# gau-nernst/pytorch-models

Measured on NVIDIA B200. Metric: ViT-B/16 img/s bf16, higher is better.
Workload: dtype bf16

## Files before the change

pytorch_models_b200/csrc/api_linear.cu:

```cuda
#include "../../include/b200enc.h"
#include "gemm.cuh"
#include "host_util.h"

using namespace b200;

namespace {

template <int kCtas, bool kFold, int kAct, bool kRes, bool kStats, bool kF8 = false, bool kPatch = false>
int launch_gemm(const CUtensorMap& ta, const CUtensorMap& tb, const CUtensorMap& tc, const GemmParams& p, int grid,
                cudaStream_t stream) {
  auto kern = gemm_bf16_kernel<kCtas, kFold, kAct, kRes, kStats, kF8, kPatch>;
  constexpr int kSmem = GemmSmem<kCtas, kRes>::kBytes;
  if (int rc = ensure_dynamic_smem(reinterpret_cast<const void*>(kern), kSmem)) return rc;
  cudaLaunchConfig_t cfg = {};
  cfg.gridDim = dim3(grid);
  cfg.blockDim = dim3(GEMM_THREADS);
  cfg.dynamicSmemBytes = kSmem;
  cfg.stream = stream;
  cudaLaunchAttribute attr[2];
  attr[0].id = cudaLaunchAttributeClusterDimension;
  attr[0].val.clusterDim.x = kCtas;
  attr[0].val.clusterDim.y = 1;
  attr[0].val.clusterDim.z = 1;
  attr[1].id = cudaLaunchAttributeProgrammaticStreamSerialization;
  attr[1].val.programmaticStreamSerializationAllowed = 1;
  cfg.attrs = attr;
  cfg.numAttrs = pdl_enabled() ? 2 : 1;
  B200_CUDA(cudaLaunchKernelEx(&cfg, kern, ta, tb, tc, p));
  return 0;
}

template <int kCtas, bool kFold, int kAct, bool kRes>
int dispatch_store(bool stats, const CUtensorMap& ta, const CUtensorMap& tb, const CUtensorMap& tc, const GemmParams& p,
                   int grid, cudaStream_t s) {
  if constexpr (kRes && !kFold) {
    if (stats) return launch_gemm<kCtas, kFold, kAct, kRes, true>(ta, tb, tc, p, grid, s);
  }
  if (stats) return set_error(-1, "b200enc_linear: stats_out needs a residual, non-folded epilogue");
  return launch_gemm<kCtas, kFold, kAct, kRes, false>(ta, tb, tc, p, grid, s);
}

template <int kCtas>
int dispatch_fp8(bool gelu, bool res, const CUtensorMap& ta, const CUtensorMap& tb, const CUtensorMap& tc, const GemmParams& p,
                 int grid, cudaStream_t s) {
  if (gelu && res) return set_error(-1, "b200enc_linear: FP8 variant: GELU and residual cannot be combined");
  if (gelu) return launch_gemm<kCtas, false, 1, false, false, true>(ta, tb, tc, p, grid, s);
  if (res) return launch_gemm<kCtas, false, 0, true, false, true>(ta, tb, tc, p, grid, s);
  return launch_gemm<kCtas, false, 0, false, false, true>(ta, tb, tc, p, grid, s);
}

template <int kCtas>
int dispatch_epilogue(int sel, bool stats, const CUtensorMap& ta, const CUtensorMap& tb,
                      const CUtensorMap& tc, const GemmParams& p, int grid, cudaStream_t s) {
  switch (sel) {
    case 0: return dispatch_store<kCtas, false, 0, false>(stats, ta, tb, tc, p, grid, s);
    case 1: return dispatch_store<kCtas, false, 0, true>(stats, ta, tb, tc, p, grid, s);
    case 2: return dispatch_store<kCtas, false, 1, false>(stats, ta, tb, tc, p, grid, s);
    case 3: return dispatch_store<kCtas, false, 1, true>(stats, ta, tb, tc, p, grid, s);
    case 4: return dispatch_store<kCtas, true, 0, false>(stats, ta, tb, tc, p, grid, s);
    case 5: return dispatch_store<kCtas, true, 0, true>(stats, ta, tb, tc, p, grid, s);
// ... 83 lines not shown
  B200_CHECK_ARG(a->ldx >= 8 && a->ldw >= K && a->ldo >= N,
                 "b200enc_linear: leading dimension smaller than the row length");
  B200_CHECK_ARG((a->colsum == nullptr) == (a->rowstats == nullptr),
                 "b200enc_linear: colsum and rowstats must be given together (LayerNorm fold)");
  if (a->colsum) {
    const int want = (K + GEMM_STAT_SLICE - 1) / GEMM_STAT_SLICE;
    B200_CHECK_ARG(a->rowstats_parts == 0 || (a->rowstats_parts == want && want <= 12),
                   "b200enc_linear: rowstats_parts=%d must be 0 or ceil(K/128)=%d (<= 12)", a->rowstats_parts, want);
  }
  B200_CHECK_ARG((reinterpret_cast<uintptr_t>(a->bias) & 15u) == 0 && (reinterpret_cast<uintptr_t>(a->colsum) & 15u) == 0,
                 "b200enc_linear: bias / colsum must be 16-byte aligned");
  if (a->residual) {
    B200_CHECK_ARG(a->ldr >= N && a->ldr % 8 == 0 && a->res_batch_stride % 8 == 0 &&
                       (reinterpret_cast<uintptr_t>(a->residual) & 15u) == 0,
                   "b200enc_linear: residual must be 16-byte aligned with strides that are multiples of 8");
  }
  const bool fold = a->colsum != nullptr;
  const bool gelu = (a->flags & B200ENC_LINEAR_GELU) != 0;
  const bool gelu_tanh = (a->flags & B200ENC_LINEAR_GELU_TANH) != 0;
  const bool relu = (a->flags & B200ENC_LINEAR_RELU) != 0;
  const bool silu = (a->flags & B200ENC_LINEAR_SILU) != 0;
  B200_CHECK_ARG(int(gelu) + int(gelu_tanh) + int(relu) + int(silu) <= 1,
                 "b200enc_linear: at most one activation flag may be set");
  constexpr int kLinearFlags =
      B200ENC_LINEAR_GELU | B200ENC_LINEAR_GELU_TANH | B200ENC_LINEAR_RELU | B200ENC_LINEAR_SILU | B200ENC_LINEAR_FP8;
  B200_CHECK_ARG((a->flags & ~kLinearFlags) == 0, "b200enc_linear: flags=%d has bits outside the documented set (0x%x)",
                 a->flags, kLinearFlags);
  const bool res = a->residual != nullptr;
  const bool stats = a->stats_out != nullptr;

  int ctas = M > GEMM_BM ? 2 : 1;
  if (ctas == 2 && K <= 1024) {
    const long long tn = (N + GEMM_BN - 1) / GEMM_BN;
    const long long t2 = (long long)((M + 2 * GEMM_BM - 1) / (2 * GEMM_BM)) * tn * batches;
    const long long t1 = (long long)((M + GEMM_BM - 1) / GEMM_BM) * tn * batches;
    const long long s2 = sm_count() / 2, s1 = sm_count();
    const double cost2 = double((t2 + s2 - 1) / s2);
    const double cost1 = double((t1 + s1 - 1) / s1) * 1.15;
    if (cost1 < cost2 * 0.97) ctas = 1;
  }
  CUtensorMap ta, tb, tc;
  int rc;
  if (fp8) {
    if ((rc = make_tmap_u8(&ta, a->x, K, M, batches, a->ldx, batches > 1 ? a->x_batch_stride : (long long)M * a->ldx,
                           2 * GEMM_BK, GEMM_BM, 128)))
      return rc;
    if ((rc = make_tmap_u8(&tb, a->w, K, N, 0, a->ldw, 0, 2 * GEMM_BK, GEMM_BN / ctas, 128))) return rc;
  } else {
    if ((rc = make_tmap_bf16(&ta, a->x, K, M, batches, a->ldx, batches > 1 ? a->x_batch_stride : (long long)M * a->ldx,
                             GEMM_BK, GEMM_BM, 128)))
      return rc;
    if ((rc = make_tmap_bf16(&tb, a->w, K, N, 0, a->ldw, 0, GEMM_BK, GEMM_BN / ctas, 128))) return rc;
  }
  if ((rc = make_tmap_bf16(&tc, a->out, N, M, batches, a->ldo,
                           batches > 1 ? a->out_batch_stride : (long long)M * a->ldo, 64, 32, 128)))
    return rc;

  GemmParams p = {};
  p.M = M;
  p.N = N;
  p.K = K;
  p.batches = batches;
  p.tiles_m = (M + GEMM_BM * ctas - 1) / (GEMM_BM * ctas);
  p.tiles_n = (N + GEMM_BN - 1) / GEMM_BN;
  p.bias = a->bias;
  p.colsum = a->colsum;
  p.rowstats = reinterpret_cast<const float2*>(a->rowstats);
  p.stat_parts = a->rowstats_parts;
  p.ln_eps = a->ln_eps;
  p.stats_out = reinterpret_cast<float2*>(a->stats_out);
  p.stats_rows = a->stats_rows_per_batch > 0 ? a->stats_rows_per_batch : M;
  p.stats_off = a->stats_row_offset;
  B200_CHECK_ARG(a->stats_row_offset >= 0 && p.stats_rows >= M + a->stats_row_offset,
                 "b200enc_linear: stats_rows_per_batch=%d cannot hold M=%d rows at offset %d", p.stats_rows, M,
                 a->stats_row_offset);
  p.res = reinterpret_cast<const __nv_bfloat16*>(a->residual);
  p.res_batch_stride = a->res_batch_stride;
  p.ldr = a->ldr;
  p.acc_scale = a->acc_scale;
  p.abort_word = abort_word();

  const long long total = (long long)p.tiles_m * p.tiles_n * batches;
  const int slots = sm_count() / ctas;
  const int grid = int(total < slots ? total : slots) * ctas;
  cudaStream_t s = reinterpret_cast<cudaStream_t>(stream);
  if (fp8) {
    if (ctas == 2) return dispatch_fp8<2>(gelu, res, ta, tb, tc, p, grid, s);
    return dispatch_fp8<1>(gelu, res, ta, tb, tc, p, grid, s);
  }
  const int sel = (silu ? 32 : 0) | (relu ? 16 : 0) | (gelu_tanh ? 8 : 0) | (fold ? 4 : 0) | (gelu ? 2 : 0) | (res ? 1 : 0);
  if (ctas == 2) return dispatch_epilogue<2>(sel, stats, ta, tb, tc, p, grid, s);
  return dispatch_epilogue<1>(sel, stats, ta, tb, tc, p, grid, s);
}
```

pytorch_models_b200/csrc/gemm.cuh:

```cuda
#pragma once
#include "ptx.cuh"

namespace b200 {

constexpr int GEMM_BM = 128;
constexpr int GEMM_BN = 256;
constexpr int GEMM_BK = 64;
constexpr int GEMM_THREADS = 320;
constexpr int GEMM_EPI_WARPS = 8;
#ifndef GEMM_STAGES_2CTA
#define GEMM_STAGES_2CTA 5
#endif
constexpr int GEMM_STAT_SLICE = 128;
constexpr int GEMM_A_BYTES = GEMM_BM * GEMM_BK * 2;
constexpr int GEMM_B_BYTES = GEMM_BN * GEMM_BK * 2;
constexpr int GEMM_STAGE_BYTES = GEMM_A_BYTES + GEMM_B_BYTES;
constexpr int GEMM_STG_BYTES = 32 * 128;
constexpr int GEMM_SMEM_COLVEC = GEMM_EPI_WARPS * 2 * 128 * 4;
template <int kCtas, bool kRes = false>
struct GemmSmem {
  static constexpr int kStages = kCtas == 2 ? (kRes ? 4 : GEMM_STAGES_2CTA) : 3;
  static constexpr int kBRows = GEMM_BN / kCtas;
  static constexpr int kStageBytes = GEMM_A_BYTES + kBRows * GEMM_BK * 2;
  static constexpr int kRing = kStages * kStageBytes;
// ... 50 lines not shown
}

__device__ __forceinline__ float2 silu_fast2(float2 x) {
  const float2 w = __fmul2_rn(x, make_float2(-1.4426950408889634f, -1.4426950408889634f));
  const float2 den = __fadd2_rn(make_float2(fast_exp2(w.x), fast_exp2(w.y)), make_float2(1.0f, 1.0f));
  return make_float2(x.x * __frcp_rn(den.x), x.y * __frcp_rn(den.y));
}

template <int kCtas, bool kFold, int kAct, bool kRes, bool kStats, bool kF8 = false, bool kPatch = false>
__global__ void __launch_bounds__(GEMM_THREADS, 1)
gemm_bf16_kernel(const __grid_constant__ CUtensorMap tmA, const __grid_constant__ CUtensorMap tmB,
                 const __grid_constant__ CUtensorMap tmC, const GemmParams p) {
  extern __shared__ __align__(1024) uint8_t smem[];
  const uint32_t smem_base = smem_u32(smem);
  using SM = GemmSmem<kCtas, kRes>;
  const uint32_t ring = smem_base;
  float* colvec = reinterpret_cast<float*>(smem + SM::kRing + SM::kStg);
  const uint32_t bars = smem_base + SM::kRing + SM::kStg + GEMM_SMEM_COLVEC;
  constexpr int kStages = SM::kStages;
  constexpr int kBRows = SM::kBRows;
  constexpr int kStageBytes = SM::kStageBytes;
  constexpr int kTileM = GEMM_BM * kCtas;
  constexpr bool kTmaOut = !kPatch;
  auto full_bar = [&](int s) { return bars + 8u * s; };
  auto empty_bar = [&](int s) { return bars + 8u * (kStages + s); };
  auto tfull_bar = [&](int a) { return bars + 8u * (2 * kStages + a); };
  auto tempty_bar = [&](int a) { return bars + 8u * (2 * kStages + 2 + a); };
  volatile uint32_t* tmem_slot = reinterpret_cast<volatile uint32_t*>(
      smem + SM::kRing + SM::kStg + GEMM_SMEM_COLVEC + 8 * (2 * kStages + 4));

  const int hw_warp = threadIdx.x >> 5;
  const int warp = (hw_warp + 2) % (GEMM_THREADS / 32);
  const int lane = threadIdx.x & 31;
  const uint32_t cta_rank = kCtas == 2 ? cluster_ctarank() : 0u;

  if (smem_base & 1023u) {
    if (threadIdx.x == 0 && p.abort_word != nullptr) *reinterpret_cast<volatile unsigned int*>(p.abort_word) = 0xB200A116u;
    return;
  }
  WaitCtx wctx = make_wait_ctx(p.abort_word);
  if (threadIdx.x == 0) {
    for (int s = 0; s < kStages; ++s) {
      mbar_init(full_bar(s), 1);
      mbar_init(empty_bar(s), 1);
    }
    for (int a = 0; a < 2; ++a) {
      mbar_init(tfull_bar(a), 1);
      mbar_init(tempty_bar(a), GEMM_EPI_WARPS * kCtas);
    }
    fence_mbar_init();
    tma_prefetch_desc(&tmA);
    tma_prefetch_desc(&tmB);
    if (kTmaOut) tma_prefetch_desc(&tmC);
  }
  if (warp == 1) {
    if (kCtas == 2) {
      tmem_alloc_2cta<512>(smem_u32(const_cast<uint32_t*>(tmem_slot)));
      tmem_relinquish_2cta();
    } else {
      tmem_alloc<512>(smem_u32(const_cast<uint32_t*>(tmem_slot)));
      tmem_relinquish();
    }
  }
  tc_fence_before();
  if (kCtas == 2) cluster_sync_all(); else __syncthreads();
  tc_fence_after();
  const uint32_t tmem_base = *tmem_slot;
  griddep_launch_dependents();
  griddep_wait();

  constexpr int kBKe = kF8 ? 2 * GEMM_BK : GEMM_BK;
  const int num_kb = (p.K + kBKe - 1) / kBKe;
  const int tiles_per_batch = p.tiles_m * p.tiles_n;
  const int total_tiles = tiles_per_batch * p.batches;
  const int first_tile = blockIdx.x / kCtas;
  const int tile_step = gridDim.x / kCtas;

  if (warp == 0) {
    uint32_t stage = 0, phase = 0;
    for (int tile = first_tile; tile < total_tiles; tile += tile_step) {
      const int b = tile / tiles_per_batch;
      const int r = tile - b * tiles_per_batch;
      const int m0 = (r / p.tiles_n) * kTileM + int(cta_rank) * GEMM_BM;
      const int n0 = (r % p.tiles_n) * GEMM_BN + int(cta_rank) * kBRows;
      for (int kb = 0; kb < num_kb; ++kb) {
        mbar_wait(empty_bar(stage), phase ^ 1u, wctx);
        const uint32_t sa = ring + stage * kStageBytes;
        if (elect_one()) {
          if (kCtas == 2) {
            const uint32_t leader_full = map_to_cta(full_bar(stage), 0);
            if (cta_rank == 0) mbar_expect_tx(full_bar(stage), 2 * kStageBytes);
            tma_load_3d_2cta(&tmA, leader_full, sa, kb * kBKe, m0, b);
            tma_load_2d_2cta(&tmB, leader_full, sa + GEMM_A_BYTES, kb * kBKe, n0);
          } else if (kPatch) {
            const int tm = r / p.tiles_n;
            mbar_expect_tx(full_bar(stage), kStageBytes);
            tma_load_4d(&tmA, full_bar(stage), sa, 0, (b * 3 + (kb >> 2)) * p.pt_hp + 8 * (tm / p.pt_nw16), (kb & 3) * 4,
                        16 * (tm % p.pt_nw16));
            tma_load_2d(&tmB, full_bar(stage), sa + GEMM_A_BYTES, kb * kBKe, n0);
          } else {
            mbar_expect_tx(full_bar(stage), kStageBytes);
            tma_load_3d(&tmA, full_bar(stage), sa, kb * kBKe, m0, b);
            tma_load_2d(&tmB, full_bar(stage), sa + GEMM_A_BYTES, kb * kBKe, n0);
          }
        }
        __syncwarp();
        if (++stage == kStages) {
          stage = 0;
          phase ^= 1u;
        }
      }
    }
  } else if (warp == 1) {
    if (cta_rank == 0) {
      constexpr uint32_t idesc = kF8 ? make_idesc_e4m3(kTileM, GEMM_BN) : make_idesc_bf16(kTileM, GEMM_BN, 0, 0);
      uint32_t stage = 0, phase = 0, acc = 0, acc_phase = 0;
      for (int tile = first_tile; tile < total_tiles; tile += tile_step) {
        mbar_wait(tempty_bar(acc), acc_phase ^ 1u, wctx);
        tc_fence_after();
        const uint32_t d_tmem = tmem_base + acc * GEMM_BN;
        for (int kb = 0; kb < num_kb; ++kb) {
          mbar_wait(full_bar(stage), phase, wctx);
          tc_fence_after();
          const uint32_t sa = ring + stage * kStageBytes;
          const uint64_t da = kPatch ? make_smem_desc_sw32(sa, 256, 1024) : make_smem_desc_sw128(sa, 16, 1024);
          constexpr uint32_t kAStep = kPatch ? 16u : 2u;
          const uint64_t db = make_smem_desc_sw128(sa + GEMM_A_BYTES, 16, 1024);
          if (elect_one()) {
#pragma unroll
            for (int k = 0; k < GEMM_BK / 16; ++k) {
              if (kF8) {
                if (kCtas == 2)
                  umma_ss_f8_2cta(d_tmem, da + kAStep * k, db + 2u * k, idesc, (kb | k) != 0 ? 1u : 0u);
                else
                  umma_ss_f8(d_tmem, da + kAStep * k, db + 2u * k, idesc, (kb | k) != 0 ? 1u : 0u);
              } else if (kCtas == 2)
                umma_ss_2cta(d_tmem, da + kAStep * k, db + 2u * k, idesc, (kb | k) != 0 ? 1u : 0u);
              else
                umma_ss(d_tmem, da + kAStep * k, db + 2u * k, idesc, (kb | k) != 0 ? 1u : 0u);
            }
            if (kCtas == 2) umma_commit_2cta(empty_bar(stage), 3); else umma_commit(empty_bar(stage));
            if (kb == num_kb - 1) {
              if (kCtas == 2) umma_commit_2cta(tfull_bar(acc), 3); else umma_commit(tfull_bar(acc));
            }
          }
          __syncwarp();
          if (++stage == kStages) {
            stage = 0;
            phase ^= 1u;
          }
        }
        acc ^= 1u;
        if (acc == 0) acc_phase ^= 1u;
      }
    }
  } else {
    const int q = hw_warp & 3;
    const int hf = (warp - 2) >> 2;
    const uint32_t stg = smem_base + SM::kRing + (warp - 2) * (SM::kStgBufs * GEMM_STG_BYTES);
    uint8_t* stg_ptr = smem + SM::kRing + (warp - 2) * (SM::kStgBufs * GEMM_STG_BYTES);
    float* cv_b = colvec + (warp - 2) * 256;
    float* cv_s = cv_b + 128;
    const int n_slices = (p.N + GEMM_STAT_SLICE - 1) / GEMM_STAT_SLICE;
    uint32_t acc = 0, acc_phase = 0;
    const uint32_t tempty_leader0 = kCtas == 2 ? map_to_cta(tempty_bar(0), 0) : tempty_bar(0);
    for (int tile = first_tile; tile < total_tiles; tile += tile_step) {
      const int b = tile / tiles_per_batch;
      const int r = tile - b * tiles_per_batch;
      const int m0 = (r / p.tiles_n) * kTileM + int(cta_rank) * GEMM_BM;
      const int n0 = (r % p.tiles_n) * GEMM_BN;
      const int pt_ph0 = kPatch ? 8 * ((r / p.tiles_n) / p.pt_nw16) : 0;
      const int pt_pw0 = kPatch ? 16 * ((r / p.tiles_n) % p.pt_nw16) : 0;
      auto tile_row = [&](int rt, bool& ok) {
        if (kPatch) {
          const int ph = pt_ph0 + (rt & 7), pw = pt_pw0 + (rt >> 3);
          ok = ph < p.pt_hp && pw < p.pt_wp;
          return ph * p.pt_wp + pw;
        }
        ok = m0 + rt < p.M;
        return m0 + rt;
      };
      bool row_ok;
      const int row = tile_row(q * 32 + lane, row_ok);
      const int nh = n0 + hf * 128;

      float4 my_b = make_float4(0.f, 0.f, 0.f, 0.f), my_s = make_float4(0.f, 0.f, 0.f, 0.f);
      if (nh + 4 * lane < p.N) {
        if (p.bias != nullptr) my_b = __ldg(reinterpret_cast<const float4*>(p.bias + nh) + lane);
        if (kFold) my_s = __ldg(reinterpret_cast<const float4*>(p.colsum + nh) + lane);
      }
      float2 st_full = make_float2(0.0f, 1.0f);
      constexpr int kMaxParts = 12;
      float2 st_part[kMaxParts];
      if (kFold && row_ok) {
        const long long grow = (long long)b * p.M + row;
        if (p.stat_parts == 0) {
          st_full = __ldg(p.rowstats + grow);
        } else {
#pragma unroll
          for (int t = 0; t < kMaxParts; ++t)
            if (t < p.stat_parts) st_part[t] = __ldg(p.rowstats + grow * p.stat_parts + t);
        }
      }
      uint4 rres[2][8];
      if (kRes) {
// ... 191 lines not shown
```

pytorch_models_b200/csrc/host_util.cu:

```cuda
#include <cstdlib>
#include "host_util.h"

#include <string.h>

#include <mutex>
#include <unordered_map>

namespace b200 {

static thread_local char g_err[512] = "";

char* last_error_buf() { return g_err; }

int set_error(int code, const char* fmt, ...) {
  va_list ap;
  va_start(ap, fmt);
  vsnprintf(g_err, sizeof(g_err), fmt, ap);
  va_end(ap);
  return code;
}

typedef CUresult (*EncodeTiledFn)(CUtensorMap*, CUtensorMapDataType, cuuint32_t, void*, const cuuint64_t*,
                                  const cuuint64_t*, const cuuint32_t*, const cuuint32_t*, CUtensorMapInterleave,
                                  CUtensorMapSwizzle, CUtensorMapL2promotion, CUtensorMapFloatOOBfill);
// ... 115 lines not shown
  if (row_stride % 16 != 0) return set_error(-1, "row stride %llu bytes is not a multiple of 16", (unsigned long long)row_stride);
  const int rank = batches == 0 ? 2 : 3;
  if (rank == 3 && batch_stride % 16 != 0)
    return set_error(-1, "batch stride %llu bytes is not a multiple of 16", (unsigned long long)batch_stride);
  const uint64_t dims[3] = {inner, rows, batches == 0 ? 1 : batches};
  const uint64_t strides[2] = {row_stride, batch_stride};
  const uint32_t box[3] = {box_inner, box_rows, 1};
  return make_tmap_bf16_nd(out, base, rank, dims, strides, box, swizzle_bytes, 1);
}

namespace {
constexpr int kMaxDevices = 64;
}

int sm_count() {
  static int counts[kMaxDevices] = {0};
  int dev = 0;
  if (cudaGetDevice(&dev) != cudaSuccess || dev < 0 || dev >= kMaxDevices) return 148;
  int n = counts[dev];
  if (n) return n;
  if (cudaDeviceGetAttribute(&n, cudaDevAttrMultiProcessorCount, dev) != cudaSuccess || n <= 0) n = 148;
  counts[dev] = n;
  return n;
}

bool pdl_enabled() {
  static const bool on = [] {
    const char* e = getenv("B200ENC_PDL");
    return !(e != nullptr && e[0] == '0');
  }();
  return on;
}

int ensure_dynamic_smem(const void* kernel, int bytes) {
  struct Key {
    const void* k;
    int dev;
    bool operator==(const Key& o) const { return k == o.k && dev == o.dev; }
  };
  struct KeyHash {
    size_t operator()(const Key& x) const { return std::hash<const void*>()(x.k) ^ (size_t(x.dev) * 0x9E3779B1u); }
  };
  static std::mutex mu;
  static std::unordered_map<Key, int, KeyHash> done;
  int dev = 0;
  B200_CUDA(cudaGetDevice(&dev));
  {
    std::lock_guard<std::mutex> lk(mu);
    auto it = done.find(Key{kernel, dev});
    if (it != done.end() && it->second >= bytes) return 0;
  }
  B200_CUDA(cudaFuncSetAttribute(kernel, cudaFuncAttributeMaxDynamicSharedMemorySize, bytes));
  std::lock_guard<std::mutex> lk(mu);
  done[Key{kernel, dev}] = bytes;
  return 0;
}

static unsigned int* g_abort_host = nullptr;

unsigned int* abort_word() {
  static std::once_flag once;
  std::call_once(once, [] {
    void* p = nullptr;
    if (cudaHostAlloc(&p, 64, cudaHostAllocMapped | cudaHostAllocPortable) == cudaSuccess && p != nullptr) {
      memset(p, 0, 64);
      g_abort_host = static_cast<unsigned int*>(p);
// ... 26 lines not shown
```

pytorch_models_b200/csrc/host_util.h:

```cpp
#pragma once
#include <cuda.h>
#include <cuda_runtime.h>
#include <stdarg.h>
#include <stdint.h>
#include <stdio.h>

namespace b200 {

char* last_error_buf();
int set_error(int code, const char* fmt, ...);

#define B200_CHECK_ARG(cond, ...)                      \
  do {                                                 \
    if (!(cond)) return b200::set_error(-1, __VA_ARGS__); \
  } while (0)

#define B200_CUDA(call)                                                                               \
  do {                                                                                                \
    cudaError_t e__ = (call);                                                                         \
    if (e__ != cudaSuccess) return b200::set_error(int(e__), "%s failed: %s", #call, cudaGetErrorString(e__)); \
  } while (0)

int make_tmap_bf16(CUtensorMap* out, const void* base, uint64_t inner, uint64_t rows, uint64_t batches,
                   uint64_t row_stride, uint64_t batch_stride, uint32_t box_inner, uint32_t box_rows,
                   int swizzle_bytes);

int make_tmap_bf16_nd(CUtensorMap* out, const void* base, int rank, const uint64_t* dims, const uint64_t* strides_bytes,
                      const uint32_t* box, int swizzle_bytes, int elem_bytes = 2);

int make_tmap_u8(CUtensorMap* out, const void* base, uint64_t inner, uint64_t rows, uint64_t batches, uint64_t row_stride,
                 uint64_t batch_stride, uint32_t box_inner, uint32_t box_rows, int swizzle_bytes);

struct TmapCacheStats {
  unsigned long long hits, misses;
};
TmapCacheStats tmap_cache_stats();

int sm_count();

int ensure_dynamic_smem(const void* kernel, int bytes);

bool pdl_enabled();

unsigned int* abort_word();
int check_abort(const char* who);
unsigned int read_abort_word(bool clear);

}
```

pytorch_models_b200/csrc/ptx.cuh:

```cuda
#pragma once
#include <cuda.h>
#include <cuda_bf16.h>
#include <cuda_runtime.h>
#include <stdint.h>
#include <stdio.h>

namespace b200 {

__device__ __forceinline__ uint32_t smem_u32(const void* p) {
  return static_cast<uint32_t>(__cvta_generic_to_shared(p));
}

__device__ __forceinline__ uint32_t lane_id() { return threadIdx.x & 31u; }

__device__ __forceinline__ bool elect_one() {
  uint32_t pred;
  asm volatile(
      "{\n\t.reg .pred p;\n\t"
      "elect.sync _|p, 0xffffffff;\n\t"
      "selp.u32 %0, 1, 0, p;\n\t}"
      : "=r"(pred));
  return pred != 0;
}

// ... 68 lines not shown
    for (int i = 0; i < 16; ++i)
      if (mbar_try_wait(bar, parity)) return;
    if ((++rounds & 63u) == 0u && w.abort_word != nullptr) {
      const uint64_t now = global_timer_ns();
      if (t0 == 0) {
        t0 = now;
      } else if (now - t0 > B200_WAIT_WATCH_NS) {
        volatile unsigned int* aw = reinterpret_cast<volatile unsigned int*>(w.abort_word);
        if (*aw != 0u) return;
        if (now - t0 > B200_WAIT_LIMIT_NS) {
          *aw = 0xB200DEADu;
          __threadfence_system();
          return;
        }
      }
    }
  }
}

__device__ __forceinline__ uint32_t lds_u32_volatile(uint32_t addr) {
  uint32_t v;
  asm volatile("ld.volatile.shared.u32 %0, [%1];" : "=r"(v) : "r"(addr) : "memory");
  return v;
}
__device__ __forceinline__ void sts_u32_volatile(uint32_t addr, uint32_t v) {
  asm volatile("st.volatile.shared.u32 [%0], %1;" ::"r"(addr), "r"(v) : "memory");
}

__device__ __forceinline__ uint32_t cluster_ctarank() {
  uint32_t r;
  asm volatile("mov.u32 %0, %%cluster_ctarank;" : "=r"(r));
  return r;
}
__device__ __forceinline__ uint32_t map_to_cta(uint32_t addr, uint32_t rank) {
  uint32_t r;
  asm volatile("mapa.shared::cluster.u32 %0, %1, %2;" : "=r"(r) : "r"(addr), "r"(rank));
  return r;
}
__device__ __forceinline__ void mbar_arrive_cluster(uint32_t cluster_addr) {
  asm volatile("mbarrier.arrive.relaxed.cluster.shared::cluster.b64 _, [%0];" ::"r"(cluster_addr) : "memory");
}
__device__ __forceinline__ void cluster_sync_all() {
  asm volatile("barrier.cluster.arrive.release.aligned;\n\tbarrier.cluster.wait.acquire.aligned;" ::: "memory");
}

__device__ __forceinline__ void fence_proxy_async_smem() {
  asm volatile("fence.proxy.async.shared::cta;" ::: "memory");
}
__device__ __forceinline__ void tc_fence_before() {
  asm volatile("tcgen05.fence::before_thread_sync;" ::: "memory");
}
__device__ __forceinline__ void tc_fence_after() {
  asm volatile("tcgen05.fence::after_thread_sync;" ::: "memory");
}

__device__ __forceinline__ void tma_prefetch_desc(const CUtensorMap* m) {
  asm volatile("prefetch.tensormap [%0];" ::"l"(reinterpret_cast<uint64_t>(m)) : "memory");
}
__device__ __forceinline__ void tma_load_2d(const CUtensorMap* m, uint32_t bar, uint32_t dst, int c0, int c1) {
  asm volatile(
      "cp.async.bulk.tensor.2d.shared::cluster.global.mbarrier::complete_tx::bytes [%0], [%1, {%3, %4}], [%2];" ::"r"(dst),
      "l"(reinterpret_cast<uint64_t>(m)), "r"(bar), "r"(c0), "r"(c1)
      : "memory");
}
__device__ __forceinline__ void tma_load_3d(const CUtensorMap* m, uint32_t bar, uint32_t dst, int c0, int c1, int c2) {
  asm volatile(
      "cp.async.bulk.tensor.3d.shared::cluster.global.mbarrier::complete_tx::bytes [%0], [%1, {%3, %4, %5}], [%2];" ::"r"(
          dst),
      "l"(reinterpret_cast<uint64_t>(m)), "r"(bar), "r"(c0), "r"(c1), "r"(c2)
      : "memory");
}
__device__ __forceinline__ void tma_load_2d_2cta(const CUtensorMap* m, uint32_t bar_cluster, uint32_t dst, int c0, int c1) {
  asm volatile(
      "cp.async.bulk.tensor.2d.cta_group::2.shared::cluster.global.mbarrier::complete_tx::bytes [%0], [%1, {%3, %4}], [%2];" ::"r"(
          dst),
      "l"(reinterpret_cast<uint64_t>(m)), "r"(bar_cluster), "r"(c0), "r"(c1)
      : "memory");
}
__device__ __forceinline__ void tma_load_3d_2cta(const CUtensorMap* m, uint32_t bar_cluster, uint32_t dst, int c0, int c1,
                                                 int c2) {
  asm volatile(
      "cp.async.bulk.tensor.3d.cta_group::2.shared::cluster.global.mbarrier::complete_tx::bytes [%0], [%1, {%3, %4, %5}], "
      "[%2];" ::"r"(dst),
      "l"(reinterpret_cast<uint64_t>(m)), "r"(bar_cluster), "r"(c0), "r"(c1), "r"(c2)
      : "memory");
}
__device__ __forceinline__ void tma_store_3d(const CUtensorMap* m, uint32_t src, int c0, int c1, int c2) {
  asm volatile("cp.async.bulk.tensor.3d.global.shared::cta.bulk_group [%0, {%2, %3, %4}], [%1];" ::"l"(
                   reinterpret_cast<uint64_t>(m)),
               "r"(src), "r"(c0), "r"(c1), "r"(c2)
               : "memory");
}
__device__ __forceinline__ void tma_store_4d(const CUtensorMap* m, uint32_t src, int c0, int c1, int c2, int c3) {
  asm volatile("cp.async.bulk.tensor.4d.global.shared::cta.bulk_group [%0, {%2, %3, %4, %5}], [%1];" ::"l"(
                   reinterpret_cast<uint64_t>(m)),
               "r"(src), "r"(c0), "r"(c1), "r"(c2), "r"(c3)
               : "memory");
}
__device__ __forceinline__ void tma_store_commit() { asm volatile("cp.async.bulk.commit_group;" ::: "memory"); }
template <int N>
__device__ __forceinline__ void tma_store_wait_read() {
  asm volatile("cp.async.bulk.wait_group.read %0;" ::"n"(N) : "memory");
}
template <int N>
__device__ __forceinline__ void tma_store_wait_all() {
  asm volatile("cp.async.bulk.wait_group %0;" ::"n"(N) : "memory");
}

template <int N>
__device__ __forceinline__ void setmaxnreg_inc() {
  asm volatile("setmaxnreg.inc.sync.aligned.u32 %0;" ::"n"(N));
}
template <int N>
__device__ __forceinline__ void setmaxnreg_dec() {
  asm volatile("setmaxnreg.dec.sync.aligned.u32 %0;" ::"n"(N));
}

// ... 183 lines not shown
```

pytorch_models_b200/csrc/selftest.cu:

```cuda
#include <cuda_bf16.h>
#include <cuda_runtime.h>
#include <math.h>
#include <stdint.h>
#include <stdio.h>
#include <stdlib.h>
#include <string.h>

#include <algorithm>
#include <string>
#include <vector>

#include "../../include/b200enc.h"

#define CK(x)                                                                         \
  do {                                                                                \
    cudaError_t e = (x);                                                              \
    if (e != cudaSuccess) {                                                           \
      printf("CUDA error %s at %s:%d: %s\n", #x, __FILE__, __LINE__, cudaGetErrorString(e)); \
      exit(3);                                                                        \
    }                                                                                 \
  } while (0)

static uint64_t g_seed = 0x9E3779B97F4A7C15ull;
static inline uint32_t rnd() {
  g_seed = g_seed * 6364136223846793005ull + 1442695040888963407ull;
  return uint32_t(g_seed >> 33);
}
static inline float urand() { return (rnd() & 0xFFFFFF) / float(0x1000000) * 2.0f - 1.0f; }

static inline uint16_t f2bf(float f) {
  uint32_t u;
  memcpy(&u, &f, 4);
  u += 0x7FFFu + ((u >> 16) & 1u);
  return uint16_t(u >> 16);
}
static inline float bf2f(uint16_t h) {
  uint32_t u = uint32_t(h) << 16;
  float f;
  memcpy(&f, &u, 4);
  return f;
}

struct DevBuf {
  void* p = nullptr;
  size_t bytes = 0;
// ... 219 lines not shown
    CK(cudaEventElapsedTime(&ms, e0, e1));
    ms /= iters;
    const double fl = 2.0 * B * double(M) * N * K;
    printf("  time %s: %.3f ms  %.1f TFLOP/s\n", c.name, ms, fl / ms * 1e-9);
    fflush(stdout);
  }
  return ok;
}

static const LinearCase kLinearCases[] = {
    {"min_tma", 1, 128, 256, 64, false, false, false, false, true, 0, 0, 0},
    {"k256_tma", 1, 128, 256, 256, false, false, false, false, true, 0, 0, 0},
    {"multi_tile", 1, 512, 768, 768, false, false, false, false, false, 0, 0, 0},
    {"tails_tma", 1, 300, 576, 192, false, false, false, false, false, 0, 0, 0},
    {"many_tiles", 1, 19000, 768, 768, false, false, false, false, false, 0, 40, 0},
    {"embed_like", 3, 196, 768, 768, false, false, true, true, false, 1, 0, 0},
    {"fold_gelu", 1, 1000, 3072, 768, true, true, false, false, false, 0, 60, 0},
    {"fold_gelu_tanh", 1, 1000, 3072, 768, true, 2, false, false, false, 0, 60, 0},
    {"gelu_tanh", 2, 300, 512, 256, false, 2, false, false, false, 0, 60, 0},
    {"relu", 2, 300, 512, 256, false, 3, false, false, false, 0, 60, 0},
    {"fold_silu", 1, 1000, 1024, 512, true, 4, false, false, false, 0, 60, 0},
    {"residual", 1, 1000, 768, 3072, false, false, true, false, false, 0, 60, 0},
    {"fold_qkv", 1, 1000, 2304, 768, true, false, false, false, false, 0, 60, 0},
    {"perf_qkv", 1, 25216, 2304, 768, true, false, false, false, false, 0, 16, 20},
    {"perf_out", 1, 25216, 768, 768, false, false, true, false, false, 0, 16, 20},
    {"perf_fc1", 1, 25216, 3072, 768, true, true, false, false, false, 0, 16, 20},
    {"perf_fc2", 1, 25216, 768, 3072, false, false, true, false, false, 0, 16, 20},
    {"perf_qkv_l2fit", 1, 8192, 2304, 768, true, false, false, false, false, 0, 16, 60},
    {"perf_qkv_big", 1, 201728, 2304, 768, true, false, false, false, false, 0, 8, 10},
    {"perf_out_big", 1, 201728, 768, 768, false, false, true, false, false, 0, 8, 10},
    {"perf_fc2_big", 1, 201728, 768, 3072, false, false, true, false, false, 0, 8, 10},
    {"perf_fc1_big", 1, 201728, 3072, 768, true, true, false, false, false, 0, 8, 10},
    {"perf_k4096", 1, 25216, 2304, 4096, false, false, false, false, false, 0, 8, 10},
};


struct AttnCase {
  const char* name;
  int B, H, Lq, Lkv;
  bool self_qkv;
  bool causal;
  float mag;
  int check_bh;
  int time_iters;
};

static bool run_attn(const AttnCase& c) {
  printf("attention %s: B=%d H=%d Lq=%d Lkv=%d self=%d causal=%d\n", c.name, c.B, c.H, c.Lq, c.Lkv, c.self_qkv,
         c.causal);
  fflush(stdout);
  const int B = c.B, H = c.H, Lq = c.Lq, Lkv = c.Lkv, D = H * 64;
  std::vector<uint16_t> hq, hkv;
  int ldq, ldkv;
  size_t koff, voff;
  if (c.self_qkv) {
    hq = rand_bf16(size_t(B) * Lq * 3 * D, c.mag, false);
    ldq = ldkv = 3 * D;
    koff = D;
    voff = 2 * D;
  } else {
    hq = rand_bf16(size_t(B) * Lq * D, c.mag, false);
    hkv = rand_bf16(size_t(B) * Lkv * 2 * D, c.mag, false);
    ldq = D;
    ldkv = 2 * D;
    koff = 0;
    voff = D;
  }
// ... 356 lines not shown
    printf("  [FAIL] %ld class-token elements were overwritten\n", untouched_bad);
    ok = false;
  }
  ok = gtok.intact("patch_embed16 tokens") && ok;
  ok = gst.intact("patch_embed16 statistics") && ok;
  if (ok && iters > 0) {
    cudaEvent_t e0, e1;
    CK(cudaEventCreate(&e0));
    CK(cudaEventCreate(&e1));
    for (int i = 0; i < 3; ++i) call();
    CK(cudaEventRecord(e0));
    for (int i = 0; i < iters; ++i) call();
    CK(cudaEventRecord(e1));
    CK(cudaEventSynchronize(e1));
    float ms = 0;
    CK(cudaEventElapsedTime(&ms, e0, e1));
    ms /= iters;
    printf("  time patch_embed16: %.3f ms  %.1f TFLOP/s  %.1f GB/s (image in, tokens out, pe)\n", ms,
           2.0 * n * P * N * K / ms * 1e-9, (2.0 * n * 3 * H * W + 2.0 * n * P * N) / ms * 1e-6);
  }
  return ok;
}

int main(int argc, char** argv) {
  if (argc < 2) {
    printf("usage: %s <case>|list\n", argv[0]);
    return 2;
  }
  std::string which = argv[1];
  if (which == "list") {
    for (auto& c : kLinearCases) printf("linear:%s\n", c.name);
    for (auto& c : kAttnCases) printf("attn:%s\n", c.name);
    printf("rows:all\n");
    return 0;
  }
  cudaDeviceProp prop;
  CK(cudaGetDeviceProperties(&prop, 0));
  printf("device: %s sm_%d%d, %d SMs\n", prop.name, prop.major, prop.minor, prop.multiProcessorCount);
  bool ok = true, found = false;
  for (auto& c : kLinearCases) {
    if (which == std::string("linear:") + c.name || which == "linear:all") {
      found = true;
      ok = run_linear(c) && ok;
    }
  }
  for (auto& c : kAttnCases) {
    if (which == std::string("attn:") + c.name || which == "attn:all") {
      found = true;
      ok = run_attn(c) && ok;
    }
  }
#ifdef ATT_TRACE
  if (which == "attn:trace") {
    found = true;
    run_attn_trace(argc > 2 ? atoi(argv[2]) : 128, argc > 3 ? atoi(argv[3]) : 12, argc > 4 ? atoi(argv[4]) : 197);
  }
#endif
  if (which == "patch:all" || which == "patch:perf") {
    found = true;
    if (which == "patch:all") {
      ok = run_patch_embed(2, 224, 224, 768, 1, true, 0) && ok;
      ok = run_patch_embed(1, 384, 384, 1024, 0, false, 0) && ok;
      ok = run_patch_embed(3, 64, 48, 256, 1, true, 0) && ok;
      ok = run_patch_embed(5, 16, 16, 64, 0, true, 0) && ok;
      ok = run_patch_embed(2, 272, 400, 384, 1, true, 0) && ok;
      ok = run_patch_embed(300, 32, 32, 128, 1, false, 0) && ok;
    } else {
      ok = run_patch_embed(1024, 224, 224, 768, 1, true, 10) && ok;
    }
  }
  if (which == "rows:all") {
    found = true;
    ok = run_layernorm(1000, 768, 1e-6f, 1, 0) && ok;
    ok = run_layernorm(333, 192, 1e-5f, 1, 0) && ok;
    ok = run_layernorm(77, 1280, 1e-5f, 1, 0) && ok;
    ok = run_layernorm(64, 1024, 1e-6f, 5, 0) && ok;
    ok = run_layernorm(201728, 768, 1e-6f, 1, 20) && ok;
    ok = run_patch(2, 224, 16, false) && ok;
    ok = run_patch(2, 224, 16, true) && ok;
    ok = run_patch(1, 518, 14, false) && ok;
    ok = run_patch(1, 518, 14, true) && ok;
    ok = run_patch(2, 64, 8, false) && ok;
  }
  if (!found) {
    printf("unknown case %s\n", which.c_str());
    return 2;
  }
  printf("%s\n", ok ? "SELFTEST PASS" : "SELFTEST FAIL");
  return ok ? 0 : 1;
}
```

Before: 29260.

## Pair 2-CTA GEMM tiles into 4-CTA clusters with multicast B loads

Launches the 2-CTA GEMM with a preferred cluster size of 4, so two adjacent CTA pairs can compute vertically neighbouring M tiles that share the same N tile. Each pair loads half of the B tile and multicasts it to the matching CTA of the other pair, which halves B-operand global/L2 traffic. To support this, the empty barriers now expect two arrivals and the MMA commits signal all four CTAs. The scheduler is reworked to walk over pairs of M tiles, and the host cost model and grid sizing are changed to match. This adds cross-pair coupling, so the two pairs proceed in lockstep. It also risks imbalance or wasted work at odd tile counts, and the fallback when the hardware forms plain 2-CTA clusters changes how B is loaded.

```diff
diff --git a/pytorch_models_b200/csrc/api_linear.cu b/pytorch_models_b200/csrc/api_linear.cu
--- a/pytorch_models_b200/csrc/api_linear.cu
+++ b/pytorch_models_b200/csrc/api_linear.cu
@@ -17,15 +17,27 @@
   cfg.blockDim = dim3(GEMM_THREADS);
   cfg.dynamicSmemBytes = kSmem;
   cfg.stream = stream;
-  cudaLaunchAttribute attr[2];
-  attr[0].id = cudaLaunchAttributeClusterDimension;
-  attr[0].val.clusterDim.x = kCtas;
-  attr[0].val.clusterDim.y = 1;
-  attr[0].val.clusterDim.z = 1;
-  attr[1].id = cudaLaunchAttributeProgrammaticStreamSerialization;
-  attr[1].val.programmaticStreamSerializationAllowed = 1;
+  cudaLaunchAttribute attr[3];
+  int n = 0;
+  attr[n].id = cudaLaunchAttributeClusterDimension;
+  attr[n].val.clusterDim.x = kCtas;
+  attr[n].val.clusterDim.y = 1;
+  attr[n].val.clusterDim.z = 1;
+  ++n;
+  if (kCtas == 2 && gemm_pair_quads()) {
+    attr[n].id = cudaLaunchAttributePreferredClusterDimension;
+    attr[n].val.preferredClusterDim.x = 4;
+    attr[n].val.preferredClusterDim.y = 1;
+    attr[n].val.preferredClusterDim.z = 1;
+    ++n;
+  }
+  if (pdl_enabled()) {
+    attr[n].id = cudaLaunchAttributeProgrammaticStreamSerialization;
+    attr[n].val.programmaticStreamSerializationAllowed = 1;
+    ++n;
+  }
   cfg.attrs = attr;
-  cfg.numAttrs = pdl_enabled() ? 2 : 1;
+  cfg.numAttrs = n;
   B200_CUDA(cudaLaunchKernelEx(&cfg, kern, ta, tb, tc, p));
   return 0;
 }
@@ -175,10 +187,10 @@
   int ctas = M > GEMM_BM ? 2 : 1;
   if (ctas == 2 && K <= 1024) {
     const long long tn = (N + GEMM_BN - 1) / GEMM_BN;
-    const long long t2 = (long long)((M + 2 * GEMM_BM - 1) / (2 * GEMM_BM)) * tn * batches;
+    const long long u2 = (long long)((M + 4 * GEMM_BM - 1) / (4 * GEMM_BM)) * tn * batches;
     const long long t1 = (long long)((M + GEMM_BM - 1) / GEMM_BM) * tn * batches;
-    const long long s2 = sm_count() / 2, s1 = sm_count();
-    const double cost2 = double((t2 + s2 - 1) / s2);
+    const long long s2 = sm_count() / 4, s1 = sm_count();
+    const double cost2 = double((u2 + s2 - 1) / s2);
     const double cost1 = double((t1 + s1 - 1) / s1) * 1.15;
     if (cost1 < cost2 * 0.97) ctas = 1;
   }
@@ -188,12 +200,12 @@
     if ((rc = make_tmap_u8(&ta, a->x, K, M, batches, a->ldx, batches > 1 ? a->x_batch_stride : (long long)M * a->ldx,
                            2 * GEMM_BK, GEMM_BM, 128)))
       return rc;
-    if ((rc = make_tmap_u8(&tb, a->w, K, N, 0, a->ldw, 0, 2 * GEMM_BK, GEMM_BN / ctas, 128))) return rc;
+    if ((rc = make_tmap_u8(&tb, a->w, K, N, 0, a->ldw, 0, 2 * GEMM_BK, ctas == 2 ? GEMM_BN / 4 : GEMM_BN, 128))) return rc;
   } else {
     if ((rc = make_tmap_bf16(&ta, a->x, K, M, batches, a->ldx, batches > 1 ? a->x_batch_stride : (long long)M * a->ldx,
                              GEMM_BK, GEMM_BM, 128)))
       return rc;
-    if ((rc = make_tmap_bf16(&tb, a->w, K, N, 0, a->ldw, 0, GEMM_BK, GEMM_BN / ctas, 128))) return rc;
+    if ((rc = make_tmap_bf16(&tb, a->w, K, N, 0, a->ldw, 0, GEMM_BK, ctas == 2 ? GEMM_BN / 4 : GEMM_BN, 128))) return rc;
   }
   if ((rc = make_tmap_bf16(&tc, a->out, N, M, batches, a->ldo,
                            batches > 1 ? a->out_batch_stride : (long long)M * a->ldo, 64, 32, 128)))
@@ -223,9 +235,10 @@
   p.acc_scale = a->acc_scale;
   p.abort_word = abort_word();
 
-  const long long total = (long long)p.tiles_m * p.tiles_n * batches;
-  const int slots = sm_count() / ctas;
-  const int grid = int(total < slots ? total : slots) * ctas;
+  const int walk = ctas == 2 ? 4 : 1;
+  const long long total = (long long)(ctas == 2 ? (p.tiles_m + 1) / 2 : p.tiles_m) * p.tiles_n * batches;
+  const int slots = sm_count() / walk;
+  const int grid = int(total < slots ? total : slots) * walk;
   cudaStream_t s = reinterpret_cast<cudaStream_t>(stream);
   if (fp8) {
     if (ctas == 2) return dispatch_fp8<2>(gelu, res, ta, tb, tc, p, grid, s);
diff --git a/pytorch_models_b200/csrc/gemm.cuh b/pytorch_models_b200/csrc/gemm.cuh
--- a/pytorch_models_b200/csrc/gemm.cuh
+++ b/pytorch_models_b200/csrc/gemm.cuh
@@ -106,7 +106,10 @@
   const int hw_warp = threadIdx.x >> 5;
   const int warp = (hw_warp + 2) % (GEMM_THREADS / 32);
   const int lane = threadIdx.x & 31;
-  const uint32_t cta_rank = kCtas == 2 ? cluster_ctarank() : 0u;
+  const uint32_t cl_rank = kCtas == 2 ? cluster_ctarank() : 0u;
+  const bool quad = kCtas == 2 && cluster_nctarank() == 4;
+  const uint32_t cta_rank = cl_rank & 1u;
+  const uint32_t leader = cl_rank & ~1u;
 
   if (smem_base & 1023u) {
     if (threadIdx.x == 0 && p.abort_word != nullptr) *reinterpret_cast<volatile unsigned int*>(p.abort_word) = 0xB200A116u;
@@ -116,7 +119,7 @@
   if (threadIdx.x == 0) {
     for (int s = 0; s < kStages; ++s) {
       mbar_init(full_bar(s), 1);
-      mbar_init(empty_bar(s), 1);
+      mbar_init(empty_bar(s), quad ? 2 : 1);
     }
     for (int a = 0; a < 2; ++a) {
       mbar_init(tfull_bar(a), 1);
@@ -145,29 +148,45 @@
 
   constexpr int kBKe = kF8 ? 2 * GEMM_BK : GEMM_BK;
   const int num_kb = (p.K + kBKe - 1) / kBKe;
-  const int tiles_per_batch = p.tiles_m * p.tiles_n;
-  const int total_tiles = tiles_per_batch * p.batches;
-  const int first_tile = blockIdx.x / kCtas;
-  const int tile_step = gridDim.x / kCtas;
+  constexpr int kWalk = kCtas == 2 ? 4 : 1;
+  const int pair_sel = kCtas == 2 ? int(blockIdx.x >> 1) & 1 : 0;
+  const int steps_m = kCtas == 2 ? (p.tiles_m + 1) >> 1 : p.tiles_m;
+  const int items_per_batch = steps_m * p.tiles_n;
+  const int total_items = items_per_batch * p.batches;
+  const int first_item = blockIdx.x / kWalk;
+  const int item_step = gridDim.x / kWalk;
+  auto item_tile = [&](int it, int& b, int& tm, int& tn) {
+    b = it / items_per_batch;
+    const int r = it - b * items_per_batch;
+    tm = (r / p.tiles_n) * (kCtas == 2 ? 2 : 1) + pair_sel;
+    tn = r % p.tiles_n;
+  };
 
   if (warp == 0) {
     uint32_t stage = 0, phase = 0;
-    for (int tile = first_tile; tile < total_tiles; tile += tile_step) {
-      const int b = tile / tiles_per_batch;
-      const int r = tile - b * tiles_per_batch;
-      const int m0 = (r / p.tiles_n) * kTileM + int(cta_rank) * GEMM_BM;
-      const int n0 = (r % p.tiles_n) * GEMM_BN + int(cta_rank) * kBRows;
+    for (int it = first_item; it < total_items; it += item_step) {
+      int b, tm, tn;
+      item_tile(it, b, tm, tn);
+      const int m0 = tm * kTileM + int(cta_rank) * GEMM_BM;
+      const int n0 = tn * GEMM_BN + int(cta_rank) * kBRows;
       for (int kb = 0; kb < num_kb; ++kb) {
         mbar_wait(empty_bar(stage), phase ^ 1u, wctx);
         const uint32_t sa = ring + stage * kStageBytes;
         if (elect_one()) {
           if (kCtas == 2) {
-            const uint32_t leader_full = map_to_cta(full_bar(stage), 0);
+            constexpr uint32_t kBHalf = kBRows / 2 * 128;
+            const uint32_t leader_full = map_to_cta(full_bar(stage), leader);
             if (cta_rank == 0) mbar_expect_tx(full_bar(stage), 2 * kStageBytes);
             tma_load_3d_2cta(&tmA, leader_full, sa, kb * kBKe, m0, b);
-            tma_load_2d_2cta(&tmB, leader_full, sa + GEMM_A_BYTES, kb * kBKe, n0);
+            if (quad) {
+              const int h = int(cl_rank >> 1);
+              tma_load_2d_2cta_mc(&tmB, leader_full, sa + GEMM_A_BYTES + h * kBHalf, kb * kBKe, n0 + h * (kBRows / 2),
+                                  uint16_t(0x5u << cta_rank));
+            } else {
+              tma_load_2d_2cta(&tmB, leader_full, sa + GEMM_A_BYTES, kb * kBKe, n0);
+              tma_load_2d_2cta(&tmB, leader_full, sa + GEMM_A_BYTES + kBHalf, kb * kBKe, n0 + kBRows / 2);
+            }
           } else if (kPatch) {
-            const int tm = r / p.tiles_n;
             mbar_expect_tx(full_bar(stage), kStageBytes);
             tma_load_4d(&tmA, full_bar(stage), sa, 0, (b * 3 + (kb >> 2)) * p.pt_hp + 8 * (tm / p.pt_nw16), (kb & 3) * 4,
                         16 * (tm % p.pt_nw16));
@@ -188,8 +207,10 @@
   } else if (warp == 1) {
     if (cta_rank == 0) {
       constexpr uint32_t idesc = kF8 ? make_idesc_e4m3(kTileM, GEMM_BN) : make_idesc_bf16(kTileM, GEMM_BN, 0, 0);
+      const uint16_t pair_mask = uint16_t(3u << leader);
+      const uint16_t empty_mask = quad ? uint16_t(0xFu) : pair_mask;
       uint32_t stage = 0, phase = 0, acc = 0, acc_phase = 0;
-      for (int tile = first_tile; tile < total_tiles; tile += tile_step) {
+      for (int it = first_item; it < total_items; it += item_step) {
         mbar_wait(tempty_bar(acc), acc_phase ^ 1u, wctx);
         tc_fence_after();
         const uint32_t d_tmem = tmem_base + acc * GEMM_BN;
@@ -213,9 +234,9 @@
               else
                 umma_ss(d_tmem, da + kAStep * k, db + 2u * k, idesc, (kb | k) != 0 ? 1u : 0u);
             }
-            if (kCtas == 2) umma_commit_2cta(empty_bar(stage), 3); else umma_commit(empty_bar(stage));
+            if (kCtas == 2) umma_commit_2cta(empty_bar(stage), empty_mask); else umma_commit(empty_bar(stage));
             if (kb == num_kb - 1) {
-              if (kCtas == 2) umma_commit_2cta(tfull_bar(acc), 3); else umma_commit(tfull_bar(acc));
+              if (kCtas == 2) umma_commit_2cta(tfull_bar(acc), pair_mask); else umma_commit(tfull_bar(acc));
             }
           }
           __syncwarp();
@@ -237,14 +258,14 @@
     float* cv_s = cv_b + 128;
     const int n_slices = (p.N + GEMM_STAT_SLICE - 1) / GEMM_STAT_SLICE;
     uint32_t acc = 0, acc_phase = 0;
-    const uint32_t tempty_leader0 = kCtas == 2 ? map_to_cta(tempty_bar(0), 0) : tempty_bar(0);
-    for (int tile = first_tile; tile < total_tiles; tile += tile_step) {
-      const int b = tile / tiles_per_batch;
-      const int r = tile - b * tiles_per_batch;
-      const int m0 = (r / p.tiles_n) * kTileM + int(cta_rank) * GEMM_BM;
-      const int n0 = (r % p.tiles_n) * GEMM_BN;
-      const int pt_ph0 = kPatch ? 8 * ((r / p.tiles_n) / p.pt_nw16) : 0;
-      const int pt_pw0 = kPatch ? 16 * ((r / p.tiles_n) % p.pt_nw16) : 0;
+    const uint32_t tempty_leader0 = kCtas == 2 ? map_to_cta(tempty_bar(0), leader) : tempty_bar(0);
+    for (int it = first_item; it < total_items; it += item_step) {
+      int b, tm, tn;
+      item_tile(it, b, tm, tn);
+      const int m0 = tm * kTileM + int(cta_rank) * GEMM_BM;
+      const int n0 = tn * GEMM_BN;
+      const int pt_ph0 = kPatch ? 8 * (tm / p.pt_nw16) : 0;
+      const int pt_pw0 = kPatch ? 16 * (tm % p.pt_nw16) : 0;
       auto tile_row = [&](int rt, bool& ok) {
         if (kPatch) {
           const int ph = pt_ph0 + (rt & 7), pw = pt_pw0 + (rt >> 3);
diff --git a/pytorch_models_b200/csrc/host_util.cu b/pytorch_models_b200/csrc/host_util.cu
--- a/pytorch_models_b200/csrc/host_util.cu
+++ b/pytorch_models_b200/csrc/host_util.cu
@@ -171,6 +171,14 @@
   return on;
 }
 
+bool gemm_pair_quads() {
+  static const bool on = [] {
+    const char* e = getenv("B200ENC_GEMM_CLUSTER");
+    return !(e != nullptr && e[0] == '2' && e[1] == '\0');
+  }();
+  return on;
+}
+
 int ensure_dynamic_smem(const void* kernel, int bytes) {
   struct Key {
     const void* k;
diff --git a/pytorch_models_b200/csrc/host_util.h b/pytorch_models_b200/csrc/host_util.h
--- a/pytorch_models_b200/csrc/host_util.h
+++ b/pytorch_models_b200/csrc/host_util.h
@@ -42,6 +42,8 @@
 
 bool pdl_enabled();
 
+bool gemm_pair_quads();
+
 unsigned int* abort_word();
 int check_abort(const char* who);
 unsigned int read_abort_word(bool clear);
diff --git a/pytorch_models_b200/csrc/ptx.cuh b/pytorch_models_b200/csrc/ptx.cuh
--- a/pytorch_models_b200/csrc/ptx.cuh
+++ b/pytorch_models_b200/csrc/ptx.cuh
@@ -124,6 +124,11 @@
   asm volatile("mov.u32 %0, %%cluster_ctarank;" : "=r"(r));
   return r;
 }
+__device__ __forceinline__ uint32_t cluster_nctarank() {
+  uint32_t r;
+  asm volatile("mov.u32 %0, %%cluster_nctarank;" : "=r"(r));
+  return r;
+}
 __device__ __forceinline__ uint32_t map_to_cta(uint32_t addr, uint32_t rank) {
   uint32_t r;
   asm volatile("mapa.shared::cluster.u32 %0, %1, %2;" : "=r"(r) : "r"(addr), "r"(rank));
@@ -175,6 +180,14 @@
       "cp.async.bulk.tensor.3d.cta_group::2.shared::cluster.global.mbarrier::complete_tx::bytes [%0], [%1, {%3, %4, %5}], "
       "[%2];" ::"r"(dst),
       "l"(reinterpret_cast<uint64_t>(m)), "r"(bar_cluster), "r"(c0), "r"(c1), "r"(c2)
+      : "memory");
+}
+__device__ __forceinline__ void tma_load_2d_2cta_mc(const CUtensorMap* m, uint32_t bar_cluster, uint32_t dst, int c0, int c1,
+                                                    uint16_t cta_mask) {
+  asm volatile(
+      "cp.async.bulk.tensor.2d.shared::cluster.global.tile.mbarrier::complete_tx::bytes.multicast::cluster.cta_group::2 "
+      "[%0], [%1, {%3, %4}], [%2], %5;" ::"r"(dst),
+      "l"(reinterpret_cast<uint64_t>(m)), "r"(bar_cluster), "r"(c0), "r"(c1), "h"(cta_mask)
       : "memory");
 }
 __device__ __forceinline__ void tma_store_3d(const CUtensorMap* m, uint32_t src, int c0, int c1, int c2) {
diff --git a/pytorch_models_b200/csrc/selftest.cu b/pytorch_models_b200/csrc/selftest.cu
--- a/pytorch_models_b200/csrc/selftest.cu
+++ b/pytorch_models_b200/csrc/selftest.cu
@@ -11,6 +11,7 @@
 #include <vector>
 
 #include "../../include/b200enc.h"
+#include "gemm.cuh"
 
 #define CK(x)                                                                         \
   do {                                                                                \
@@ -296,7 +297,89 @@
     {"perf_fc2_big", 1, 201728, 768, 3072, false, false, true, false, false, 0, 8, 10},
     {"perf_fc1_big", 1, 201728, 3072, 768, true, true, false, false, false, 0, 8, 10},
     {"perf_k4096", 1, 25216, 2304, 4096, false, false, false, false, false, 0, 8, 10},
+    {"quad_odd_res", 3, 600, 768, 200, false, false, true, false, false, 0, 0, 0},
+    {"quad_odd_fold_gelu", 2, 1100, 3072, 768, true, true, false, false, false, 0, 0, 0},
+    {"quad_odd_qkv", 2, 700, 2304, 776, true, false, false, false, false, 0, 0, 0},
+    {"quad_one_unit", 1, 300, 256, 136, false, false, true, true, false, 0, 0, 0},
 };
+
+static __global__ void __launch_bounds__(320, 1) placement_probe(int* rec, unsigned long long hold_ns) {
+  extern __shared__ uint8_t probe_smem[];
+  unsigned r, n, sm;
+  asm volatile("mov.u32 %0, %%cluster_ctarank;" : "=r"(r));
+  asm volatile("mov.u32 %0, %%cluster_nctarank;" : "=r"(n));
+  asm volatile("mov.u32 %0, %%smid;" : "=r"(sm));
+  if (threadIdx.x == 0) {
+    probe_smem[0] = 1;
+    rec[3 * blockIdx.x] = int(r);
+    rec[3 * blockIdx.x + 1] = int(n);
+    rec[3 * blockIdx.x + 2] = int(sm);
+    unsigned long long t0, t;
+    asm volatile("mov.u64 %0, %%globaltimer;" : "=l"(t0));
+    do {
+      asm volatile("mov.u64 %0, %%globaltimer;" : "=l"(t));
+    } while (t - t0 < hold_ns);
+  }
+}
+
+static bool run_placement() {
+  constexpr int kSmem = b200::GemmSmem<2, false>::kBytes;
+  static_assert(kSmem == b200::GemmSmem<2, true>::kBytes, "both pair-tile smem plans are probed as one");
+  int dev = 0, nsm = 0;
+  CK(cudaGetDevice(&dev));
+  CK(cudaDeviceGetAttribute(&nsm, cudaDevAttrMultiProcessorCount, dev));
+  CK(cudaFuncSetAttribute(placement_probe, cudaFuncAttributeMaxDynamicSharedMemorySize, kSmem));
+  const int grid = nsm / 4 * 4;
+  cudaLaunchConfig_t cfg = {};
+  cfg.gridDim = dim3(grid);
+  cfg.blockDim = dim3(320);
+  cfg.dynamicSmemBytes = kSmem;
+  cudaLaunchAttribute attr[2];
+  attr[0].id = cudaLaunchAttributeClusterDimension;
+  attr[0].val.clusterDim.x = 2;
+  attr[0].val.clusterDim.y = 1;
+  attr[0].val.clusterDim.z = 1;
+  cfg.attrs = attr;
+  cfg.numAttrs = 1;
+  for (int cl : {2, 4}) {
+    attr[0].val.clusterDim.x = cl;
+    int n = 0;
+    CK(cudaOccupancyMaxActiveClusters(&n, placement_probe, &cfg));
+    printf("  cudaOccupancyMaxActiveClusters, cluster %d, %d B shared memory: %d (%d CTAs)\n", cl, kSmem, n, n * cl);
+  }
+  attr[0].val.clusterDim.x = 2;
+  attr[1].id = cudaLaunchAttributePreferredClusterDimension;
+  attr[1].val.preferredClusterDim.x = 4;
+  attr[1].val.preferredClusterDim.y = 1;
+  attr[1].val.preferredClusterDim.z = 1;
+  cfg.numAttrs = 2;
+  DevBuf rec(size_t(grid) * 3 * 4);
+  CK(cudaLaunchKernelEx(&cfg, placement_probe, (int*)rec.p, 200000ull));
+  CK(cudaDeviceSynchronize());
+  std::vector<int> h(size_t(grid) * 3);
+  CK(cudaMemcpy(h.data(), rec.p, h.size() * 4, cudaMemcpyDeviceToHost));
+  std::vector<int> sm_used(4096, 0);
+  int quads = 0, pairs = 0, bad = 0, distinct = 0;
+  for (int j = 0; j < grid / 4; ++j) {
+    const int* q = &h[size_t(12) * j];
+    const int n = q[1];
+    bool ok = n == 4 || n == 2;
+    for (int i = 0; i < 4; ++i) ok = ok && q[3 * i + 1] == n && q[3 * i] == (n == 4 ? i : (i & 1));
+    if (!ok) {
+      if (bad++ < 8)
+        printf("  quad %d: (rank, size) = (%d,%d) (%d,%d) (%d,%d) (%d,%d)\n", j, q[0], q[1], q[3], q[4], q[6], q[7], q[9],
+               q[10]);
+    }
+    (n == 4 ? quads : pairs) += 1;
+  }
+  for (int b = 0; b < grid; ++b) {
+    const int sm = h[size_t(3) * b + 2];
+    if (sm >= 0 && sm < 4096 && sm_used[sm]++ == 0) ++distinct;
+  }
+  printf("  grid %d on %d SMs: %d block quads formed one 4-CTA cluster, %d ran as two pairs, %d misaligned; "
+         "%d distinct SMs\n", grid, nsm, quads, pairs, bad, distinct);
+  return bad == 0 && distinct == grid;
+}
 
 
 struct AttnCase {
@@ -719,6 +802,7 @@
     for (auto& c : kLinearCases) printf("linear:%s\n", c.name);
     for (auto& c : kAttnCases) printf("attn:%s\n", c.name);
     printf("rows:all\n");
+    printf("gemm:placement\n");
     return 0;
   }
   cudaDeviceProp prop;
@@ -756,6 +840,10 @@
       ok = run_patch_embed(1024, 224, 224, 768, 1, true, 10) && ok;
     }
   }
+  if (which == "gemm:placement") {
+    found = true;
+    ok = run_placement() && ok;
+  }
   if (which == "rows:all") {
     found = true;
     ok = run_layernorm(1000, 768, 1e-6f, 1, 0) && ok;
```

Result: no change. 29510 (median of 6 runs) (+0.9%).
